# GMC-DRL/MetaBox

Hardware: AMD Instinct MI355X
Metric: env-steps/sec (instances x gens/s), RLEPSO bbob-easy d=10 (higher is better)
Workload: dtype f64

## Files before the change

include/mbx.h:

```cpp
#ifndef MBX_H
#define MBX_H

#include <stddef.h>
#include <stdint.h>

#ifdef __cplusplus
extern "C" {
#endif

#define MBX_OK            0
#define MBX_E_ARG        -1
#define MBX_E_HIP        -2
#define MBX_E_UNSUPPORTED -3
#define MBX_E_NOMEM      -4

#define MBX_KIND_PROTEIN 100

#define MBX_NOISE_NONE    0
#define MBX_NOISE_GAUSS   1
#define MBX_NOISE_UNIFORM 2
#define MBX_NOISE_CAUCHY  3

typedef struct mbx_problem_desc {
    int32_t func_id;
// ... 134 lines not shown
    const float* d_weights;
    int32_t n_floats;
    float min_sigma, max_sigma;
} mbx_gleet_actor;
int mbx_gleet_policy(mbx_batch* b, const mbx_gleet_actor* net, const double* d_state, float* d_actions, float* d_mu_sigma, void* stream);

int mbx_qlpso_rollout(mbx_batch* b, const double* d_q_table, int n_steps, int32_t* d_actions_out, double* d_state_out,
                      double* d_reward_out, uint8_t* d_done_out, void* stream);

int mbx_debug_math(int op, const double* d_x, const double* d_y, double* d_out, int n, void* stream);

int mbx_debug_rlepso_draws(uint64_t seed, int gen, int episode, int np, int dim, double* d_out, void* stream);

int mbx_batch_launch_info(const mbx_batch* b, int32_t out[4]);

int mbx_debug_clock_probe(uint64_t* d_out, int n_samples, int sleep_units, void* stream);
int mbx_debug_clock_mark(uint64_t* d_out2, void* stream);
int mbx_debug_clock_slots(mbx_batch* b, uint64_t* d_slots2);

const char* mbx_last_error(void);
const char* mbx_version(void);

#ifdef __cplusplus
}
#endif
#endif
```

metabox_amd/_abi.py:

```python
import ctypes as C
import os

import numpy as np

_HERE = os.path.dirname(os.path.abspath(__file__))
LIB_PATH = os.environ.get('MBX_LIB') or os.path.join(_HERE, 'csrc', 'libmbx.so')

c_double_p = C.POINTER(C.c_double)


class ProblemDesc(C.Structure):
    _fields_ = [('func_id', C.c_int32), ('kind', C.c_int32), ('dim', C.c_int32), ('n_peaks', C.c_int32),
                ('noise_kind', C.c_int32), ('reserved', C.c_int32),
                ('bias', C.c_double), ('lb', C.c_double), ('ub', C.c_double), ('pen_coef', C.c_double),
                ('s', C.c_double * 4), ('noise_a', C.c_double), ('noise_b', C.c_double),
                ('dshift', c_double_p), ('m1', c_double_p), ('m2', c_double_p),
                ('v0', c_double_p), ('v1', c_double_p), ('v2', c_double_p),
                ('py', c_double_p), ('pc', c_double_p), ('pw', c_double_p)]


class AlgoCfg(C.Structure):
    _fields_ = [('algo', C.c_int32), ('np', C.c_int32), ('dim', C.c_int32), ('max_fes', C.c_int32),
                ('log_interval', C.c_int32), ('n_logpoint', C.c_int32), ('early_stop', C.c_int32),
                ('n_group', C.c_int32), ('flags', C.c_uint32)]
# ... 52 lines not shown
    keep = []
    for i, d in enumerate(descs):
        st, k = pack_desc(d)
        arr[i] = st
        keep.extend(k)
    return arr, keep


_lib = None


class MbxError(RuntimeError):
    pass


def load_lib():
    global _lib
    if _lib is not None:
        return _lib
    if not os.path.exists(LIB_PATH) and not os.environ.get('MBX_LIB'):
        import shutil
        import subprocess
        if shutil.which('hipcc') or os.path.exists('/opt/rocm/bin/hipcc'):
            subprocess.call(['make', '-C', os.path.join(_HERE, 'csrc'), '-s'])
    if not os.path.exists(LIB_PATH):
        raise MbxError(f'{LIB_PATH} is missing: build it with `python -c "import __graft_entry__ as g; g.build()"` '
                       f'(hipcc --offload-arch=gfx950). metabox_amd has no CPU fallback.')
    lib = C.CDLL(LIB_PATH)
    vp, i32, u64, i64 = C.c_void_p, C.c_int32, C.c_uint64, C.c_int64
    proto = {
# ... 18 lines not shown
        'mbx_lde_policy': (C.c_int, [vp, C.POINTER(LstmPolicy), vp, vp, vp, vp, vp, vp]),
        'mbx_ddqn_qnet': (C.c_int, [vp, C.POINTER(QNet), vp, vp, vp, vp]),
        'mbx_rlepso_policy_table_rows': (C.c_int, [vp]),
        'mbx_rlepso_policy_table': (C.c_int, [vp, C.POINTER(GaussMlp), vp, vp]),
        'mbx_rlepso_act_step': (C.c_int, [vp, vp, vp, vp, vp, vp, vp]),
        'mbx_rlepso_rollout_resident': (C.c_int, [vp]),
        'mbx_rlepso_rollout': (C.c_int, [vp, vp, C.c_int, vp, vp, vp, vp, vp, vp, vp, vp]),
        'mbx_lde_rollout_resident': (C.c_int, [vp]),
        'mbx_lde_rollout': (C.c_int, [vp, C.POINTER(LstmPolicy), vp, vp, vp, C.c_int, vp, vp, vp, vp, vp, vp, vp, vp]),
        'mbx_rlpso_rollout': (C.c_int, [vp, C.POINTER(GaussMlp), C.c_int, vp, vp, vp, vp, vp]),
        'mbx_qlpso_rollout': (C.c_int, [vp, vp, C.c_int, vp, vp, vp, vp, vp]),
        'mbx_gleet_policy': (C.c_int, [vp, C.POINTER(GleetActor), vp, vp, vp, vp]),
        'mbx_debug_math': (C.c_int, [C.c_int, vp, vp, vp, C.c_int, vp]),
        'mbx_debug_rlepso_draws': (C.c_int, [C.c_uint64, C.c_int, C.c_int, C.c_int, C.c_int, vp, vp]),
        'mbx_batch_launch_info': (C.c_int, [vp, C.POINTER(C.c_int32)]),
        'mbx_instance_state_doubles': (i64, [vp]),
        'mbx_debug_read_state': (C.c_int, [vp, C.c_int, c_double_p]),
        'mbx_debug_write_state': (C.c_int, [vp, C.c_int, c_double_p]),
        'mbx_debug_clock_probe': (C.c_int, [vp, C.c_int, C.c_int, vp]),
        'mbx_debug_clock_mark': (C.c_int, [vp, vp]),
        'mbx_debug_clock_slots': (C.c_int, [vp, vp]),
        'mbx_batch_rebind': (C.c_int, [vp, vp, vp]),
        'mbx_read_public': (C.c_int, [vp, C.c_int, c_double_p, vp]),
        'mbx_last_error': (C.c_char_p, []),
        'mbx_version': (C.c_char_p, []),
    }
    for name, (res, args) in proto.items():
        fn = getattr(lib, name)
        fn.restype = res
        fn.argtypes = args
    _lib = lib
    return lib


EXPORTED_SYMBOLS = ('mbx_suite_create', 'mbx_suite_destroy', 'mbx_suite_size', 'mbx_suite_optimum', 'mbx_suite_close_pairs', 'mbx_eval', 'mbx_state_dim', 'mbx_action_dim',
                    'mbx_tape_stride', 'mbx_batch_create', 'mbx_batch_destroy', 'mbx_batch_flags', 'mbx_set_tape', 'mbx_reset', 'mbx_step', 'mbx_results',
                    'mbx_gauss_policy', 'mbx_lde_policy', 'mbx_ddqn_qnet', 'mbx_rlepso_policy_table_rows', 'mbx_rlepso_policy_table', 'mbx_rlepso_act_step',
                    'mbx_rlepso_rollout_resident', 'mbx_rlepso_rollout', 'mbx_lde_rollout_resident', 'mbx_lde_rollout', 'mbx_rlpso_rollout',
                    'mbx_qlpso_rollout', 'mbx_gleet_policy', 'mbx_debug_math', 'mbx_debug_rlepso_draws', 'mbx_batch_launch_info', 'mbx_instance_state_doubles',
                    'mbx_debug_read_state', 'mbx_debug_write_state', 'mbx_debug_clock_probe', 'mbx_debug_clock_mark', 'mbx_debug_clock_slots',
                    'mbx_batch_rebind', 'mbx_read_public', 'mbx_last_error', 'mbx_version')


def check(rc):
    if rc != 0:
        msg = load_lib().mbx_last_error()
        raise MbxError(f'mbx error {rc}: {msg.decode() if msg else "?"}')
```

metabox_amd/csrc/mbx.hip:

```cpp
#include <hip/hip_runtime.h>

#include <cmath>
#include <cstdarg>
#include <cstdio>
#include <cstring>
#include <algorithm>
#include <memory>
#include <string>
#include <vector>

#include "mbx_device.hpp"
#include "mbx_rlepso.hpp"
#include "mbx_lde.hpp"
#ifndef MBX_LDE100_STEP_THREADS
#define MBX_LDE100_STEP_THREADS 512
#endif
#ifndef MBX_LDE50_STEP_THREADS
#define MBX_LDE50_STEP_THREADS 256
#endif
#include "mbx_ddqn.hpp"
#include "mbx_rs.hpp"
#include "mbx_policy.hpp"
#include "mbx_lstm_policy.hpp"
#include "mbx_lde_run.hpp"
// ... 935 lines not shown
}

extern "C" int mbx_rlepso_rollout_resident(const mbx_batch* b)
{
    if (!b) return fail(MBX_E_ARG, "mbx_rlepso_rollout_resident: null batch");
    if (b->cfg.algo != MBX_ALGO_RLEPSO) return 0;
    return (b->fixed_geometry == 1 || b->fixed_geometry == 2 || b->fixed_geometry == 7 || b->fixed_geometry == 8 || b->fixed_geometry == 10) && !b->rollout_per_generation ? 1 : 0;
}

__global__ void k_sum_rewards(double* __restrict__ acc, const double* __restrict__ r, int n, int first)
{
    const int i = blockIdx.x * blockDim.x + threadIdx.x;
    if (i < n) acc[i] = first ? r[i] : acc[i] + r[i];
}

static int launch_rlepso_run(mbx_batch* b, const float* d_table, int rows, int n_gens, const RunOut& out, hipStream_t stream)
{
#define MBX_RUN_LAUNCH(T, ...) hipLaunchKernelGGL((k_rlepso_run<T, __VA_ARGS__>), dim3(b->B), dim3(T), b->lds_bytes, stream, make_params(b), d_table, rows, n_gens, out)
    if (b->fixed_geometry == 1) { if (b->fdr_fast) MBX_RUN_LAUNCH(MBX_RUN10_THREADS, 100, 10, 5, false); else MBX_RUN_LAUNCH(MBX_RUN10_THREADS, 100, 10, 5, true); }
    else if (b->fixed_geometry == 2) { if (b->fdr_fast) MBX_RUN_LAUNCH(1024, 128, 40, 5, false); else MBX_RUN_LAUNCH(1024, 128, 40, 5, true); }
    else if (b->fixed_geometry == 7) MBX_RUN_LAUNCH(512, 100, 30, 5, true);
    else if (b->fixed_geometry == 8) MBX_RUN_LAUNCH(256, 100, 12, 5, true);
    else if (b->fixed_geometry == 10) MBX_RUN_LAUNCH(1024, 100, 40, 5, true);
    else return fail(MBX_E_UNSUPPORTED, "k_rlepso_run: no instantiation for this geometry");
#undef MBX_RUN_LAUNCH
    HIP_TRY(hipGetLastError());
    return MBX_OK;
}

extern "C" int mbx_rlepso_rollout(mbx_batch* b, const float* d_table, int n_gens, float* d_traj_actions, double* d_traj_state,
                                  double* d_traj_reward, uint8_t* d_traj_done, double* d_state_out, double* d_reward_out,
                                  uint8_t* d_done_out, void* stream)
{
// ... 230 lines not shown
    b->d_clk = (unsigned long long*)d_slots2;
    return MBX_OK;
}

extern "C" int mbx_batch_launch_info(const mbx_batch* b, int32_t out[4])
{
    if (!b || !out) return fail(MBX_E_ARG, "mbx_batch_launch_info: bad arguments");
    out[0] = b->threads; out[1] = (int32_t)b->lds_bytes; out[2] = b->fixed_geometry; out[3] = (int32_t)b->state_stride;
    if (b->cfg.algo == MBX_ALGO_LDE && b->fixed_geometry == 3) out[0] = MBX_LDE50_STEP_THREADS;
    if (b->cfg.algo == MBX_ALGO_DEDDQN) {
        out[0] = kDqStepThreads; out[1] = (int32_t)(dq_lds_doubles(1, b->cfg.np, b->cfg.dim) * sizeof(double));
    }
    return MBX_OK;
}

extern "C" int mbx_debug_math(int op, const double* d_x, const double* d_y, double* d_out, int n, void* stream)
{
    if (op < 0 || op > 6 || !d_x || !d_out || n < 0 || ((op == 4 || op == 6) && !d_y)) return fail(MBX_E_ARG, "mbx_debug_math: bad arguments");
    if (n) hipLaunchKernelGGL(k_debug_math, dim3((n + 255) / 256), dim3(256), 0, (hipStream_t)stream, op, d_x, d_y, d_out, n);
    HIP_TRY(hipGetLastError());
    return MBX_OK;
}

extern "C" int64_t mbx_instance_state_doubles(const mbx_batch* b)
{
    if (!b) return fail(MBX_E_ARG, "null batch");
    return geom_of(b->cfg).state_doubles;
}

extern "C" int mbx_debug_read_state(mbx_batch* b, int instance, double* host_out)
// ... 44 lines not shown
```

metabox_amd/csrc/mbx_device.hpp:

```cpp
#pragma once
#include <type_traits>
#include <hip/hip_runtime.h>
#include <stdint.h>

#include "../../include/mbx.h"
#include "../../include/mbx_layout.h"
#include "mbx_math.hpp"

namespace mbx {

#ifdef MBX_NOINLINE_MATH
#define MBX_MATH __device__ __noinline__
#else
#define MBX_MATH __device__ __forceinline__
#endif
#ifdef MBX_LIBM_MATH
MBX_MATH double m_pow(double a, double b) { return pow(a, b); }
MBX_MATH double m_sin(double a) { return sin(a); }
MBX_MATH double m_cos(double a) { return cos(a); }
MBX_MATH double m_exp(double a) { return exp(a); }
MBX_MATH double m_log(double a) { return log(a); }
#else
MBX_MATH double m_pow(double a, double b) { return fm::pow_fast(a, b); }
MBX_MATH double m_sin(double a) { return fm::sincos_fast<false>(a); }
// ... 195 lines not shown
__device__ __forceinline__ double asy1(double x, double beta_lin)
{
    return x > 0. ? m_pow(x, 1. + beta_lin * sqrt(x)) : x;
}

__device__ __forceinline__ double pen_row(const double* x, int D, double ub)
{
    double s = 0.;
    for (int d = 0; d < D; ++d) {
        const double t = fmax(0., fabs(x[d]) - ub);
        s += t * t;
    }
    return s;
}

__host__ __device__ inline long long eval_t_doubles(int n, int D)
{
    long long t = (long long)n * D;
    if (t < 17ll * D) t = 17ll * D;
    if (t < 8ll * n) t = 8ll * n;
    return (t + 1) & ~1ll;
}

struct EvalLds {
    const double* X;
    double *Z, *T;
    double *M1T, *M2T;
    double *DSH, *V0, *V1, *V2;
    double* F;
    int z_doubles = 0;
};
// ... 837 lines not shown
```

metabox_amd/csrc/mbx_rlepso.hpp:

```cpp
#pragma once
#include "mbx_device.hpp"

namespace mbx {

struct BatchParams {
    const DevProblem* problems;
    const int32_t* problem_idx;
    const uint64_t* seeds;
    double* state;
    int64_t state_stride;
    const double* tape;
    int64_t tape_stride;
    const int32_t* order;
    const double* pci;
    int32_t NP, D, max_fes, log_interval, n_logpoint, early_stop, n_group, B;
    int64_t sc_off;
    unsigned long long* clk;
};

template <class PT>
__device__ __forceinline__ bool log_and_terminate(const BatchParams& bp, const PT& P, double fes, double gbest, int& log_index,
                                                  int& cost_len, double* __restrict__ cost)
{
    if (fes >= (double)log_index * bp.log_interval) { log_index += 1; cost[cost_len++] = gbest; }
    bool done = fes >= bp.max_fes;
    if (!isnan(P.optimum) && bp.early_stop) done = done || gbest <= 1e-8;
    if (done) {
        if (cost_len >= bp.n_logpoint + 1) cost[cost_len - 1] = gbest;
        else cost[cost_len++] = gbest;
    }
    return done;
}

struct RlLds {
    double *PB, *X, *Z, *T, *M1T, *M2T, *DSH, *V0, *V1, *V2, *PBC, *NC, *PNI, *CMUT, *R1, *R2, *GB, *COEF, *RED;
    int *IMPR, *MASK, *RANK;
    uint8_t* KB;
    uint16_t* FL;
    int* FLN;
    double* NCS;
    int zd;
    __device__ __forceinline__ EvalLds eval() const { return EvalLds{X, Z, T, M1T, M2T, DSH, V0, V1, V2, NC, zd}; }
};

__host__ __device__ inline int64_t align2(int64_t n) { return (n + 1) & ~(int64_t)1; }

__host__ __device__ inline int64_t rl_aux_doubles(int NP, int D) { const int64_t NE = (int64_t)NP * D; return ((NE + 15) / 16 * 16 + 16 + 2 * NE + 7) / 8; }

__host__ __device__ inline int64_t rl_z_doubles(int NP, int D)
{
    const int64_t NE = align2((int64_t)NP * D);
    int64_t need = 3 * align2(NP) + 96 + rl_aux_doubles(NP, D);
    if (need < 2 * kThreads) need = 2 * kThreads;
    if (D == 12 && need < 4 * 4 * 100) need = 4 * 4 * 100;
    return align2(NE > need ? NE : need);
}

#ifndef MBX_RUN_KC40
#define MBX_RUN_KC40 8
#endif
#ifndef MBX_RUN_KC30
#define MBX_RUN_KC30 0
#endif
__host__ __device__ constexpr int rl_run_matvec_chunk(int D) { return D == 40 ? MBX_RUN_KC40 : D == 30 ? MBX_RUN_KC30 : 0; }

__host__ __device__ constexpr bool rl_maps_in_lds(int NP, int D) { return !(NP == 100 && D == 30); }

// ... 25 lines not shown
    L.V0 = p; p += align2(D);
    L.V1 = p; p += align2(D);
    L.V2 = p; p += align2(D);
    L.PBC = p; p += P;
    L.NC = p; p += P;
    L.PNI = p; p += P;
    L.CMUT = p; p += P;
    L.GB = p; p += align2(D);
    L.RED = p; p += 16;
    L.IMPR = (int*)p; p += align2((P + 1) / 2);
    L.MASK = (int*)p; p += align2((P + 1) / 2);
    L.RANK = (int*)p;
    return L;
}

__device__ __forceinline__ void rl_commit(const RlLds& L, int NP, int D, bool stagnation, double& gbest, int& gbest_idx,
                                          double* __restrict__ gPB, double* __restrict__ gCC)
{
    const int tid = threadIdx.x;
    for (int i = tid; i < NP; i += MBX_NT) {
        const double nc = L.NC[i];
        if (stagnation) L.PNI[i] = nc < gCC[i] ? 0. : L.PNI[i] + 1;
        const int impr = nc < L.PBC[i];
        if (impr) L.PBC[i] = nc;
        L.IMPR[i] = impr;
        gCC[i] = nc;
    }
    double cbv; int cb;
    block_argmin(L.NC, NP, L.RED, cbv, cb);
    const bool better = cbv < gbest;
// ... 291 lines not shown
        if (others[q]) {
            double qb = aw[q] / bw[q];
            int ib = ORDER[kb[q]];
            for (int k = 0; k < nless; ++k) {
                const double a = NC[k] - fi, b = fabs(PB[k * D + d0 + q] - pp[q]) + 1e-5, pr = aw[q] * b;
                if (__builtin_fma(a, bw[q], -pr) <= pr * -0x1p-49 && k != kw[q] && !(a == aw[q] && b == bw[q])) {
                    const double qk = a / b;
                    const int ik = ORDER[k];
                    if (qk < qb || (qk == qb && ik < ib)) { qb = qk; ib = ik; kb[q] = k; }
                }
            }
        }
    }
}

template <int W, int UN, bool TIE, int THREADS>
__device__ __forceinline__ void fdr_pass(const RlLds& L, const int* ORDER, const int* NLESS, int NP, int D, int tid, double range, unsigned long long* cnt = nullptr)
{
    const int DW = D / W, NI = NP * DW;
    const FastDiv fw(DW);
    uint32_t mine = 0;
    for (int base = 0, pass = 0; base < NI; base += THREADS, ++pass) {
        const int lim = base + THREADS < NI ? base + THREADS : NI;
        const int ps = (pass & 1) ? lim - 1 - tid : base + tid;
        if (ps >= base && ps < lim) {
            const int rk = fw.div(ps), d0 = W * (ps - rk * DW);
            int kb[W];
            const bool tie = fdr_exact<W, UN, TIE>(L, D, rk, d0, NLESS[ORDER[rk]], kb, range);
#pragma unroll
            for (int q = 0; q < W; ++q) L.KB[rk * D + d0 + q] = (uint8_t)kb[q];
#ifdef MBX_FDR_COUNT
            if (cnt) { atomicAdd(cnt + 3, 1ull); if (tie) atomicAdd(cnt + 2, 1ull); }
#endif
            if (TIE && tie) { L.FL[atomicAdd(L.FLN, 1)] = (uint16_t)ps; mine |= 1u << (pass & 31); }
        }
    }
    __syncthreads();
    if constexpr (TIE) {
        const int n = *L.FLN;
        if (n > 0 && (n <= MBX_FDR_OWN_AT || NI > 32 * THREADS)) {
            for (int c = tid >> 6; c < W * n; c += THREADS / 64) {
                const int ps = L.FL[c / W], rk = fw.div(ps), d = W * (ps - rk * DW) + c % W;
                const int kbest = fdr_settle(L, ORDER, D, rk, d, NLESS[ORDER[rk]], L.KB[rk * D + d], cnt);
                if ((tid & 63) == 0) L.KB[rk * D + d] = (uint8_t)kbest;
            }
            __syncthreads();
        } else if (n > 0) {
            for (int base = 0, pass = 0; mine != 0u; base += THREADS, ++pass, mine >>= 1) {
                if (!(mine & 1u)) continue;
                const int lim = base + THREADS < NI ? base + THREADS : NI;
                const int ps = (pass & 1) ? lim - 1 - tid : base + tid, rk = fw.div(ps), d0 = W * (ps - rk * DW);
// ... 337 lines not shown
        if (done_out) done_out[b] = done ? 1 : 0;
    }
    MBX_PHASE(8);
}

struct RunOut {
    float* traj_actions;
    double* traj_state;
    double* traj_reward;
    uint8_t* traj_done;
    double* state_out;
    double* reward_out;
    uint8_t* done_out;
};

#ifndef MBX_RUN_WAVES
#define MBX_RUN_WAVES MBX_RL_WAVES
#endif
template <int THREADS, int NPC, int DC, int GC, int KIND, int NOISE, bool TIE, class ARGS>
__device__ __forceinline__ void rl_run_body(ARGS ar)
{
    const int n_gens = ar().n_gens;
    static_assert(NPC > 0 && DC > 0 && GC > 0 && (DC & 1) == 0 && NPC <= THREADS, "k_rlepso_run: compile-time geometry, even D, NP <= THREADS");
    constexpr int NP = NPC, D = DC, G = GC, HD = D / 2, NI = NP * HD, IT = (NI + THREADS - 1) / THREADS, A = 7 * G;
    extern __shared__ __attribute__((aligned(16))) double smem[];
    const int b = ar().bp.order[blockIdx.x], tid0 = threadIdx.x, tid = tid0;
    double* S = ar().bp.state + (int64_t)b * ar().bp.state_stride;
    double* sc = S + MBX_RLEPSO_ST_SCALARS(NP, D);
    const int64_t B = ar().bp.B;

    if (sc[MBX_SC_DONE] != 0.) {
        const double st = sc[MBX_SC_FES] / ar().bp.max_fes;
        for (int g = tid; g < n_gens; g += THREADS) {
            if (ar().out.traj_state) ar().out.traj_state[g * B + b] = st;
            if (ar().out.traj_reward) ar().out.traj_reward[g * B + b] = 0.;
            if (ar().out.traj_done) ar().out.traj_done[g * B + b] = 1;
        }
        if (tid == 0) {
            if (ar().out.state_out) ar().out.state_out[b] = st;
            if (ar().out.reward_out) ar().out.reward_out[b] = 0.;
            if (ar().out.done_out) ar().out.done_out[b] = 1;
        }
        return;
    }
    unsigned long long clk_c0 = 0, clk_r0 = 0;
    const bool clocked = ar().bp.clk != nullptr && tid0 == 0;
    if (clocked) { clk_c0 = __builtin_amdgcn_s_memtime(); clk_r0 = __builtin_amdgcn_s_memrealtime(); }
    ConstProblem& P = *(ConstProblem*)(ar().bp.problems + ar().bp.problem_idx[b]);
    const RlLds L = rl_carve(smem, NP, D, rl_maps_in_lds(NPC, DC));
    int gen = (int)sc[MBX_SC_GEN];
    const uint64_t seed = ar().bp.seeds[b];
    const uint32_t episode = (uint32_t)(int)sc[MBX_SC_EPISODE];
    const double lb = P.lb, ub = P.ub, vmax = 0.1 * (ub - lb);
    double gbest = sc[MBX_SC_GBEST];
    int gbest_idx = (int)sc[MBX_SC_GBEST_IDX];
    double fes = sc[MBX_SC_FES];
    int log_index = (int)sc[MBX_SC_LOG_INDEX], cost_len = (int)sc[MBX_SC_COST_LEN];
    double* cost = sc + MBX_NSCALAR;
    double ret = 0.;
    int n_reinit = 0;

    double* gPos = S + MBX_RLEPSO_ST_POS(NP, D);
    double* gVel = S + MBX_RLEPSO_ST_VEL(NP, D);
    double* gPB = S + MBX_RLEPSO_ST_PBPOS(NP, D);
    double vel[IT][2], pbp[IT][2], cc = 0.;
#pragma unroll
    for (int j = 0; j < IT; ++j) {
        const int it = tid + j * THREADS;
        vel[j][0] = vel[j][1] = pbp[j][0] = pbp[j][1] = 0.;
        if (it < NI) {
            const double2 v2 = *(const double2*)(gVel + 2 * it), p2 = *(const double2*)(gPB + 2 * it);
            vel[j][0] = v2.x; vel[j][1] = v2.y; pbp[j][0] = p2.x; pbp[j][1] = p2.y;
            *(double2*)(L.X + 2 * it) = *(const double2*)(gPos + 2 * it);
        }
    }
    if (tid < NP) {
        L.PBC[tid] = S[MBX_RLEPSO_ST_PBEST(NP, D) + tid];
        L.PNI[tid] = S[MBX_RLEPSO_ST_PNI(NP, D) + tid];
        cc = S[MBX_RLEPSO_ST_CCOST(NP, D) + tid];
    }
    if (tid < D) L.GB[tid] = S[MBX_RLEPSO_ST_GBPOS(NP, D) + tid];
    stage_problem<eval_dc(DC), eval_md(DC) == 0, ConstProblem>(P, L.eval());
    constexpr int per_group = NP / G;
    const FastDiv fg(per_group), fh(HD);
    int* ORDER = L.IMPR;
    int* NLESS = L.MASK;
    int* RANK = L.RANK;
    float* ACT = (float*)L.R1;
    int* EQC = (int*)(L.RED + 14);

    auto commit = [&](bool stagnation, int tid) {
        if (tid < NP) {
            const double nc = L.NC[tid];
            if (stagnation) L.PNI[tid] = nc < cc ? 0. : L.PNI[tid] + 1;
            const int impr = nc < L.PBC[tid];
            if (impr) L.PBC[tid] = nc;
            L.IMPR[tid] = impr;
            cc = nc;
        }
        double cbv; int cb;
        block_argmin(L.NC, NP, L.RED, cbv, cb);
        const bool better = cbv < gbest;
        if (better) { gbest = cbv; gbest_idx = cb; }
#pragma unroll
        for (int j = 0; j < IT; ++j) {
            const int it = tid + j * THREADS;
            if (it < NI && L.IMPR[fh.div(it)]) { const double2 x2 = *(const double2*)(L.X + 2 * it); pbp[j][0] = x2.x; pbp[j][1] = x2.y; }
        }
        if (better && tid < D) L.GB[tid] = L.X[cb * D + tid];
        __syncthreads();
    };

    bool done = false;
    int g = 0;
    __syncthreads();
    for (; g < n_gens && !done; ++g) {
        int tid = tid0;
        asm volatile("" : "+v"(tid));
        gen += 1;
        const Rng rng{(uint32_t)seed, (uint32_t)(seed >> 32), (uint32_t)gen, episode, true};
        const double pre_gbest = gbest;
        if (tid < A) {
            int row = (int)fes;
            row = row < ar().table_rows ? row : ar().table_rows - 1;
            const float* ms = ar().policy_table + (int64_t)row * 2 * A;
            const float a = sample_action(rng, tid, ms[tid], ms[A + tid], MBX_POLICY_RLEPSO);
            ACT[tid] = a;
            if (ar().out.traj_actions) ar().out.traj_actions[((int64_t)g * B + b) * A + tid] = a;
        }
        if (tid < NP) { NLESS[tid] = 0; ORDER[tid] = tid; }
        if (tid == 0) { *EQC = 0; *L.FLN = 0; }
        __syncthreads();
        if (tid < G) {
            const float* a = ACT + tid * G;
            const float cm = a[0] * 0.01f;
            const float wv = a[1] * 0.8f + 0.1f;
            float den = a[3] + a[4];
            den = den + a[5]; den = den + a[6]; den = den + 1e-5f;
            float scale = 1.f / den;
            scale = scale * a[2]; scale = scale * 8.f;
            double* c = L.COEF + tid * 6;
            c[0] = (double)cm; c[1] = (double)wv;
            c[2] = (double)(scale * a[3]); c[3] = (double)(scale * a[4]);
            c[4] = (double)(scale * a[5]); c[5] = (double)(scale * a[6]);
        }
        {
            constexpr int parts = THREADS / NP > 0 ? THREADS / NP : 1;
            for (int w = tid; w < parts * NP; w += THREADS) {
                const int part = w / NP, i = w - part * NP;
                const int j0 = part * NP / parts, j1 = (part + 1) * NP / parts;
                const double fi = L.PBC[i];
                int nless = 0;
#ifndef MBX_ABLATE_RANK
#pragma unroll 5
                for (int j = j0; j < j1; ++j) nless += L.PBC[j] < fi;
#else
                if (part == 0) nless = i;
#endif
                atomicAdd(&NLESS[i], nless);
            }
        }
        __syncthreads();
        if (tid < NP) {
            const int i = tid, gi = fg.div(i);
            L.CMUT[i] = gi < G ? L.COEF[gi * 6] * L.PNI[i] : 0.;
            const U4 w = rng.draw((uint32_t)i, MBX_SITE_PART);
            L.R1[i] = u53(w.x, w.y); L.R2[i] = u53(w.z, w.w);
            const int rank = NLESS[i];
            RANK[i] = rank;
            ORDER[rank] = i; L.NC[rank] = L.PBC[i]; L.NCS[rank] = L.PBC[i];
        }
        __syncthreads();
        if (tid < NP && ORDER[RANK[tid]] != tid) *EQC = 1;
        auto stage_pbest = [&](int tid) {
#pragma unroll
            for (int j = 0; j < IT; ++j) {
                const int it = tid + j * THREADS;
                if (it < NI) { const int i = fh.div(it), d0 = 2 * (it - i * HD); *(double2*)(L.PB + RANK[i] * D + d0) = double2{pbp[j][0], pbp[j][1]}; }
            }
        };
        stage_pbest(tid);
        __syncthreads();
        if (*EQC) {
            int rank = 0;
            if (tid < NP) {
                const double fi = L.PBC[tid];
                rank = NLESS[tid];
                for (int j = 0; j < tid; ++j) rank += L.PBC[j] == fi;
            }
            __syncthreads();
            if (tid < NP) { RANK[tid] = rank; ORDER[rank] = tid; L.NC[rank] = L.PBC[tid]; L.NCS[rank] = L.PBC[tid]; }
            __syncthreads();
            stage_pbest(tid);
            __syncthreads();
            rl_mark_copies(L, NP, D, tid);
            __syncthreads();
        }
#ifdef MBX_ABLATE_FDR
        for (int e = tid; e < NP * D; e += THREADS) L.KB[e] = 0;
        __syncthreads();
#else
        fdr_pass<2, (DC == 40 ? 2 : MBX_FDR_UNROLL), TIE, THREADS>(L, ORDER, NLESS, NP, D, tid, ub - lb + 1e-5, ar().bp.clk);
#endif
        {
            const MoveCtx mc{L, ar().bp.pci, nullptr, rng, nullptr, nullptr, ORDER, NLESS, RANK, NP, D, G, lb, ub, vmax, fg};
#pragma unroll
            for (int j = 0; j < IT; ++j) {
                const int it = tid + j * THREADS;
                if (it < NI) {
                    const int i = fh.div(it);
                    const double2 c2 = *(const double2*)(L.X + 2 * it);
                    double cur[2] = {c2.x, c2.y};
                    rl_move<2, true>(mc, i, 2 * (it - i * HD), cur, vel[j]);
                }
            }
        }
        __syncthreads();
        population_costs<eval_dc(DC), eval_md(DC), ConstProblem, rl_run_matvec_chunk(DC), KIND, NOISE>(P, L.eval(), NP, rng, nullptr, MBX_SITE_NOISE0_A, MBX_SITE_NOISE0_B);
        fes += NP;
        commit(true, tid);
        int mine = 0;
        if (tid < NP) {
            const U4 w = rng.draw((uint32_t)tid, MBX_SITE_REINIT);
            const double u = u53(w.x, w.y);
            mine = u < L.CMUT[tid] * 0.01 * L.PNI[tid];
            L.MASK[tid] = mine;
        }
        n_reinit = __syncthreads_count(mine);
        if (n_reinit > 0) {
#pragma unroll
            for (int j = 0; j < IT; ++j) {
                const int it = tid + j * THREADS;
                if (it < NI && L.MASK[fh.div(it)]) {
#pragma unroll
                    for (int q = 0; q < 2; ++q) {
                        const int e = 2 * it + q;
                        const U4 w = rng.draw((uint32_t)e, MBX_SITE_ELEM_R);
                        const double up = u53(w.x, w.y), uv = u53(w.z, w.w);
                        L.X[e] = lb + (ub - lb) * up;
                        vel[j][q] = -vmax + (vmax - (-vmax)) * uv;
                    }
                }
            }
            __syncthreads();
            population_costs<eval_dc(DC), eval_md(DC), ConstProblem, rl_run_matvec_chunk(DC), KIND, NOISE>(P, L.eval(), NP, rng, nullptr, MBX_SITE_NOISE1_A, MBX_SITE_NOISE1_B);
            fes += n_reinit;
            commit(false, tid);
        }
        if (fes >= (double)log_index * ar().bp.log_interval) { log_index += 1; if (tid == 0) cost[cost_len] = gbest; cost_len += 1; }
        done = fes >= ar().bp.max_fes;
        if (!isnan(P.optimum) && ar().bp.early_stop) done = done || gbest <= 1e-8;
        if (done) {
            if (cost_len >= ar().bp.n_logpoint + 1) { if (tid == 0) cost[cost_len - 1] = gbest; }
            else { if (tid == 0) cost[cost_len] = gbest; cost_len += 1; }
        }
        const double reward = gbest < pre_gbest ? 1. : -1.;
        ret += reward;
        if (tid == 0) {
            if (ar().out.traj_state) ar().out.traj_state[g * B + b] = fes / ar().bp.max_fes;
            if (ar().out.traj_reward) ar().out.traj_reward[g * B + b] = reward;
            if (ar().out.traj_done) ar().out.traj_done[g * B + b] = done ? 1 : 0;
        }
    }
#pragma unroll
    for (int j = 0; j < IT; ++j) {
        const int it = tid + j * THREADS;
        if (it < NI) {
            *(double2*)(gPos + 2 * it) = *(const double2*)(L.X + 2 * it);
            *(double2*)(gVel + 2 * it) = double2{vel[j][0], vel[j][1]};
            *(double2*)(gPB + 2 * it) = double2{pbp[j][0], pbp[j][1]};
        }
    }
    if (tid < NP) {
        S[MBX_RLEPSO_ST_PBEST(NP, D) + tid] = L.PBC[tid];
        S[MBX_RLEPSO_ST_PNI(NP, D) + tid] = L.PNI[tid];
        S[MBX_RLEPSO_ST_CCOST(NP, D) + tid] = cc;
    }
    if (tid < D) S[MBX_RLEPSO_ST_GBPOS(NP, D) + tid] = L.GB[tid];
    const double st = fes / ar().bp.max_fes;
    for (int t = g + tid; t < n_gens; t += THREADS) {
        if (ar().out.traj_state) ar().out.traj_state[t * B + b] = st;
        if (ar().out.traj_reward) ar().out.traj_reward[t * B + b] = 0.;
        if (ar().out.traj_done) ar().out.traj_done[t * B + b] = 1;
    }
    if (tid == 0) {
        sc[MBX_SC_GBEST] = gbest; sc[MBX_SC_FES] = fes; sc[MBX_SC_LOG_INDEX] = log_index; sc[MBX_SC_COST_LEN] = cost_len;
        sc[MBX_SC_DONE] = done ? 1. : 0.; sc[MBX_SC_RETURN] += ret; sc[MBX_SC_GEN] = gen;
        sc[MBX_SC_GBEST_IDX] = gbest_idx; sc[MBX_SC_REINIT] = n_reinit > 0 ? 1. : 0.;
        if (ar().out.state_out) ar().out.state_out[b] = st;
        if (ar().out.reward_out) ar().out.reward_out[b] = ret;
// ... 74 lines not shown
```

metabox_amd/suite.py:

```python
import ctypes as C

import numpy as np
import torch

from . import _abi


def _require_gpu():
    if not torch.cuda.is_available():
        raise _abi.MbxError('metabox_amd needs a ROCm GPU (MI355X); there is no CPU fallback for the hot path.')


def _ptr(t):
    return C.c_void_p(t.data_ptr()) if t is not None else C.c_void_p()


def _stream():
    return C.c_void_p(torch.cuda.current_stream().cuda_stream)


class Suite:

    def __init__(self, problems):
        _require_gpu()
# ... 273 lines not shown
        _abi.check(self.lib.mbx_debug_read_state(self._h, int(instance), out.ctypes.data_as(_abi.c_double_p)))
        return out

    def write_state(self, instance, block):
        n = int(self.lib.mbx_instance_state_doubles(self._h))
        block = np.ascontiguousarray(block, dtype=np.float64)
        assert block.shape == (n,)
        _abi.check(self.lib.mbx_debug_write_state(self._h, int(instance), block.ctypes.data_as(_abi.c_double_p)))

    def launch_info(self):
        import ctypes as C
        out = (C.c_int32 * 4)()
        _abi.check(self.lib.mbx_batch_launch_info(self._h, out))
        return {'threads': out[0], 'lds_bytes': out[1], 'fixed_geometry': out[2], 'state_doubles': out[3]}

    def close(self):
        if getattr(self, '_h', None):
            self.lib.mbx_batch_destroy(self._h)
            self._h = None

    def __del__(self):
        try:
            self.close()
        except Exception:
            pass
```

Baseline: 35.67 million.

## Compact LDS and park velocity/pbest in global memory for six RLEPSO workgroups per CU

For the 256-thread, NP=100, D=10 resident RLEPSO kernel, this adds a compact LDS carve-out. It drops the matrix maps, CMUT and the double PNI array, and stores integer tables in the free tail of Z. Velocity and personal-best positions move out of registers into global memory, and the velocity fetch is hooked into the FDR pass so it overlaps. The waves-per-EU hint rises to 6, aiming for six workgroups per CU to raise occupancy. In exchange it adds global memory traffic each generation and re-reads maps from global memory instead of LDS, and it adds an occupancy-query diagnostic API.

```diff
diff --git a/include/mbx.h b/include/mbx.h
--- a/include/mbx.h
+++ b/include/mbx.h
@@ -172,6 +172,8 @@
 
 int mbx_batch_launch_info(const mbx_batch* b, int32_t out[4]);
 
+int mbx_rlepso_run_launch_info(const mbx_batch* b, int32_t out[3]);
+
 int mbx_debug_clock_probe(uint64_t* d_out, int n_samples, int sleep_units, void* stream);
 int mbx_debug_clock_mark(uint64_t* d_out2, void* stream);
 int mbx_debug_clock_slots(mbx_batch* b, uint64_t* d_slots2);
diff --git a/metabox_amd/_abi.py b/metabox_amd/_abi.py
--- a/metabox_amd/_abi.py
+++ b/metabox_amd/_abi.py
@@ -90,6 +90,9 @@
     pass
 
 
+_DIAGNOSTICS_SINCE = ('mbx_rlepso_run_launch_info',)
+
+
 def load_lib():
     global _lib
     if _lib is not None:
@@ -138,6 +141,7 @@
         'mbx_debug_math': (C.c_int, [C.c_int, vp, vp, vp, C.c_int, vp]),
         'mbx_debug_rlepso_draws': (C.c_int, [C.c_uint64, C.c_int, C.c_int, C.c_int, C.c_int, vp, vp]),
         'mbx_batch_launch_info': (C.c_int, [vp, C.POINTER(C.c_int32)]),
+        'mbx_rlepso_run_launch_info': (C.c_int, [vp, C.POINTER(C.c_int32)]),
         'mbx_instance_state_doubles': (i64, [vp]),
         'mbx_debug_read_state': (C.c_int, [vp, C.c_int, c_double_p]),
         'mbx_debug_write_state': (C.c_int, [vp, C.c_int, c_double_p]),
@@ -150,6 +154,8 @@
         'mbx_version': (C.c_char_p, []),
     }
     for name, (res, args) in proto.items():
+        if name in _DIAGNOSTICS_SINCE and os.environ.get('MBX_LIB') and not hasattr(lib, name):
+            continue
         fn = getattr(lib, name)
         fn.restype = res
         fn.argtypes = args
@@ -161,7 +167,8 @@
                     'mbx_tape_stride', 'mbx_batch_create', 'mbx_batch_destroy', 'mbx_batch_flags', 'mbx_set_tape', 'mbx_reset', 'mbx_step', 'mbx_results',
                     'mbx_gauss_policy', 'mbx_lde_policy', 'mbx_ddqn_qnet', 'mbx_rlepso_policy_table_rows', 'mbx_rlepso_policy_table', 'mbx_rlepso_act_step',
                     'mbx_rlepso_rollout_resident', 'mbx_rlepso_rollout', 'mbx_lde_rollout_resident', 'mbx_lde_rollout', 'mbx_rlpso_rollout',
-                    'mbx_qlpso_rollout', 'mbx_gleet_policy', 'mbx_debug_math', 'mbx_debug_rlepso_draws', 'mbx_batch_launch_info', 'mbx_instance_state_doubles',
+                    'mbx_qlpso_rollout', 'mbx_gleet_policy', 'mbx_debug_math', 'mbx_debug_rlepso_draws', 'mbx_batch_launch_info', 'mbx_rlepso_run_launch_info',
+                    'mbx_instance_state_doubles',
                     'mbx_debug_read_state', 'mbx_debug_write_state', 'mbx_debug_clock_probe', 'mbx_debug_clock_mark', 'mbx_debug_clock_slots',
                     'mbx_batch_rebind', 'mbx_read_public', 'mbx_last_error', 'mbx_version')
 
diff --git a/metabox_amd/csrc/mbx.hip b/metabox_amd/csrc/mbx.hip
--- a/metabox_amd/csrc/mbx.hip
+++ b/metabox_amd/csrc/mbx.hip
@@ -973,9 +973,17 @@
     if (i < n) acc[i] = first ? r[i] : acc[i] + r[i];
 }
 
+static size_t rlepso_run_lds_bytes(const mbx_batch* b)
+{
+    if (b->fixed_geometry == 1 && rl_run_compact(MBX_RUN10_THREADS, 100, 10))
+        return (size_t)rl_run_lds_doubles(100, 10) * sizeof(double) + (b->lds_bytes - (size_t)rl_lds_doubles(100, 10, true) * sizeof(double));
+    return b->lds_bytes;
+}
+
 static int launch_rlepso_run(mbx_batch* b, const float* d_table, int rows, int n_gens, const RunOut& out, hipStream_t stream)
 {
-#define MBX_RUN_LAUNCH(T, ...) hipLaunchKernelGGL((k_rlepso_run<T, __VA_ARGS__>), dim3(b->B), dim3(T), b->lds_bytes, stream, make_params(b), d_table, rows, n_gens, out)
+    const size_t run_lds = rlepso_run_lds_bytes(b);
+#define MBX_RUN_LAUNCH(T, ...) hipLaunchKernelGGL((k_rlepso_run<T, __VA_ARGS__>), dim3(b->B), dim3(T), run_lds, stream, make_params(b), d_table, rows, n_gens, out)
     if (b->fixed_geometry == 1) { if (b->fdr_fast) MBX_RUN_LAUNCH(MBX_RUN10_THREADS, 100, 10, 5, false); else MBX_RUN_LAUNCH(MBX_RUN10_THREADS, 100, 10, 5, true); }
     else if (b->fixed_geometry == 2) { if (b->fdr_fast) MBX_RUN_LAUNCH(1024, 128, 40, 5, false); else MBX_RUN_LAUNCH(1024, 128, 40, 5, true); }
     else if (b->fixed_geometry == 7) MBX_RUN_LAUNCH(512, 100, 30, 5, true);
@@ -1236,6 +1244,27 @@
     return MBX_OK;
 }
 
+extern "C" int mbx_rlepso_run_launch_info(const mbx_batch* b, int32_t out[3])
+{
+    if (!b || !out) return fail(MBX_E_ARG, "mbx_rlepso_run_launch_info: bad arguments");
+    if (mbx_rlepso_rollout_resident(b) != 1) return fail(MBX_E_UNSUPPORTED, "mbx_rlepso_run_launch_info: the batch's rollout does not take the resident kernel");
+    const void* k = nullptr;
+    int threads = 0;
+#define MBX_RUN_KERNEL(T, ...) do { k = (const void*)k_rlepso_run<T, __VA_ARGS__>; threads = T; } while (0)
+    if (b->fixed_geometry == 1) { if (b->fdr_fast) MBX_RUN_KERNEL(MBX_RUN10_THREADS, 100, 10, 5, false); else MBX_RUN_KERNEL(MBX_RUN10_THREADS, 100, 10, 5, true); }
+    else if (b->fixed_geometry == 2) { if (b->fdr_fast) MBX_RUN_KERNEL(1024, 128, 40, 5, false); else MBX_RUN_KERNEL(1024, 128, 40, 5, true); }
+    else if (b->fixed_geometry == 7) MBX_RUN_KERNEL(512, 100, 30, 5, true);
+    else if (b->fixed_geometry == 8) MBX_RUN_KERNEL(256, 100, 12, 5, true);
+    else if (b->fixed_geometry == 10) MBX_RUN_KERNEL(1024, 100, 40, 5, true);
+    else return fail(MBX_E_UNSUPPORTED, "k_rlepso_run: no instantiation for this geometry");
+#undef MBX_RUN_KERNEL
+    const size_t lds = rlepso_run_lds_bytes(b);
+    int per_cu = 0;
+    HIP_TRY(hipOccupancyMaxActiveBlocksPerMultiprocessor(&per_cu, k, threads, lds));
+    out[0] = threads; out[1] = (int32_t)lds; out[2] = per_cu;
+    return MBX_OK;
+}
+
 extern "C" int mbx_debug_math(int op, const double* d_x, const double* d_y, double* d_out, int n, void* stream)
 {
     if (op < 0 || op > 6 || !d_x || !d_out || n < 0 || ((op == 4 || op == 6) && !d_y)) return fail(MBX_E_ARG, "mbx_debug_math: bad arguments");
diff --git a/metabox_amd/csrc/mbx_device.hpp b/metabox_amd/csrc/mbx_device.hpp
--- a/metabox_amd/csrc/mbx_device.hpp
+++ b/metabox_amd/csrc/mbx_device.hpp
@@ -233,7 +233,7 @@
     return s;
 }
 
-__host__ __device__ inline long long eval_t_doubles(int n, int D)
+__host__ __device__ constexpr long long eval_t_doubles(int n, int D)
 {
     long long t = (long long)n * D;
     if (t < 17ll * D) t = 17ll * D;
diff --git a/metabox_amd/csrc/mbx_rlepso.hpp b/metabox_amd/csrc/mbx_rlepso.hpp
--- a/metabox_amd/csrc/mbx_rlepso.hpp
+++ b/metabox_amd/csrc/mbx_rlepso.hpp
@@ -35,6 +35,7 @@
 struct RlLds {
     double *PB, *X, *Z, *T, *M1T, *M2T, *DSH, *V0, *V1, *V2, *PBC, *NC, *PNI, *CMUT, *R1, *R2, *GB, *COEF, *RED;
     int *IMPR, *MASK, *RANK;
+    int* PNII = nullptr;
     uint8_t* KB;
     uint16_t* FL;
     int* FLN;
@@ -43,14 +44,16 @@
     __device__ __forceinline__ EvalLds eval() const { return EvalLds{X, Z, T, M1T, M2T, DSH, V0, V1, V2, NC, zd}; }
 };
 
-__host__ __device__ inline int64_t align2(int64_t n) { return (n + 1) & ~(int64_t)1; }
-
-__host__ __device__ inline int64_t rl_aux_doubles(int NP, int D) { const int64_t NE = (int64_t)NP * D; return ((NE + 15) / 16 * 16 + 16 + 2 * NE + 7) / 8; }
-
-__host__ __device__ inline int64_t rl_z_doubles(int NP, int D)
+__host__ __device__ constexpr int64_t align2(int64_t n) { return (n + 1) & ~(int64_t)1; }
+
+__host__ __device__ constexpr int64_t rl_aux_doubles(int NP, int D) { const int64_t NE = (int64_t)NP * D; return ((NE + 15) / 16 * 16 + 16 + 2 * NE + 7) / 8; }
+
+__host__ __device__ constexpr int64_t rl_z_move_doubles(int NP, int D) { return 3 * align2(NP) + 96 + rl_aux_doubles(NP, D); }
+
+__host__ __device__ constexpr int64_t rl_z_doubles(int NP, int D)
 {
     const int64_t NE = align2((int64_t)NP * D);
-    int64_t need = 3 * align2(NP) + 96 + rl_aux_doubles(NP, D);
+    int64_t need = rl_z_move_doubles(NP, D);
     if (need < 2 * kThreads) need = 2 * kThreads;
     if (D == 12 && need < 4 * 4 * 100) need = 4 * 4 * 100;
     return align2(NE > need ? NE : need);
@@ -106,6 +109,49 @@
     return L;
 }
 
+#ifndef MBX_RUN_COMPACT
+#define MBX_RUN_COMPACT 1
+#endif
+#ifndef MBX_LDS_GRANULE
+#define MBX_LDS_GRANULE 1280
+#endif
+__host__ __device__ constexpr bool rl_run_compact(int THREADS, int NP, int D) { return MBX_RUN_COMPACT && THREADS == 256 && NP == 100 && D == 10; }
+
+__host__ __device__ constexpr int64_t rl_run_lds_doubles(int NP, int D)
+{
+    const int64_t NE = align2((int64_t)NP * D), P = align2(NP);
+    return eval_t_doubles(NP, D) + NE + rl_z_doubles(NP, D) + 5 * align2(D) + 2 * P + 16 + align2((P + 1) / 2);
+}
+
+__device__ __forceinline__ RlLds rl_carve_run(double* base, int NP, int D)
+{
+    const int64_t NE = align2((int64_t)NP * D), SC = rl_z_doubles(NP, D), P = align2(NP), TS = eval_t_doubles(NP, D), IT = align2((P + 1) / 2);
+    RlLds L;
+    double* p = base;
+    L.PB = p; L.T = p; p += TS;
+    L.X = p; p += NE;
+    L.Z = p; L.zd = (int)SC;
+    L.R1 = p; L.R2 = p + P; L.COEF = p + 2 * P;
+    L.NCS = p + 2 * P + 96;
+    L.KB = (uint8_t*)(p + 3 * P + 96);
+    L.FLN = (int*)(L.KB + ((int64_t)NP * D + 15) / 16 * 16);
+    L.FL = (uint16_t*)(L.FLN + 4);
+    double* tail = p + rl_z_move_doubles(NP, D);
+    L.MASK = (int*)tail; L.RANK = (int*)(tail + IT); L.IMPR = (int*)(tail + 2 * IT);
+    p += SC;
+    L.M1T = nullptr; L.M2T = nullptr; L.PNI = nullptr; L.CMUT = nullptr;
+    L.DSH = p; p += align2(D);
+    L.V0 = p; p += align2(D);
+    L.V1 = p; p += align2(D);
+    L.V2 = p; p += align2(D);
+    L.GB = p; p += align2(D);
+    L.PBC = p; p += P;
+    L.NC = p; p += P;
+    L.RED = p; p += 16;
+    L.PNII = (int*)p;
+    return L;
+}
+
 __device__ __forceinline__ void rl_commit(const RlLds& L, int NP, int D, bool stagnation, double& gbest, int& gbest_idx,
                                           double* __restrict__ gPB, double* __restrict__ gCC)
 {
@@ -427,8 +473,10 @@
     }
 }
 
-template <int W, int UN, bool TIE, int THREADS>
-__device__ __forceinline__ void fdr_pass(const RlLds& L, const int* ORDER, const int* NLESS, int NP, int D, int tid, double range, unsigned long long* cnt = nullptr)
+struct FdrNoHook { __device__ __forceinline__ void operator()() const {} };
+template <int W, int UN, bool TIE, int THREADS, class HOOK = FdrNoHook>
+__device__ __forceinline__ void fdr_pass(const RlLds& L, const int* ORDER, const int* NLESS, int NP, int D, int tid, double range, unsigned long long* cnt = nullptr,
+                                         HOOK after_scan = HOOK())
 {
     const int DW = D / W, NI = NP * DW;
     const FastDiv fw(DW);
@@ -448,6 +496,7 @@
             if (TIE && tie) { L.FL[atomicAdd(L.FLN, 1)] = (uint16_t)ps; mine |= 1u << (pass & 31); }
         }
     }
+    after_scan();
     __syncthreads();
     if constexpr (TIE) {
         const int n = *L.FLN;
@@ -815,15 +864,27 @@
     uint8_t* done_out;
 };
 
+#ifndef MBX_RUN_SIX
+#define MBX_RUN_SIX 1
+#endif
 #ifndef MBX_RUN_WAVES
-#define MBX_RUN_WAVES MBX_RL_WAVES
-#endif
+#define MBX_RUN_WAVES __attribute__((amdgpu_waves_per_eu(MBX_RUN_SIX && rl_run_compact(THREADS, NPC, DC) ? 6 : THREADS == 256 ? 5 : 4)))
+#endif
+#ifndef MBX_RUN_PARK
+#define MBX_RUN_PARK 1
+#endif
+__host__ __device__ constexpr bool rl_run_parked(int THREADS, int NP, int D) { return MBX_RUN_PARK && THREADS == 256 && NP == 100 && D == 10; }
 template <int THREADS, int NPC, int DC, int GC, int KIND, int NOISE, bool TIE, class ARGS>
 __device__ __forceinline__ void rl_run_body(ARGS ar)
 {
     const int n_gens = ar().n_gens;
     static_assert(NPC > 0 && DC > 0 && GC > 0 && (DC & 1) == 0 && NPC <= THREADS, "k_rlepso_run: compile-time geometry, even D, NP <= THREADS");
     constexpr int NP = NPC, D = DC, G = GC, HD = D / 2, NI = NP * HD, IT = (NI + THREADS - 1) / THREADS, A = 7 * G;
+    constexpr bool PARK = rl_run_parked(THREADS, NPC, DC);
+    constexpr bool COMPACT = rl_run_compact(THREADS, NPC, DC);
+    constexpr int MDR = COMPACT ? DC : eval_md(DC);
+    static_assert(!COMPACT || rl_z_move_doubles(NPC, DC) + 3 * align2((align2(NPC) + 1) / 2) <= rl_z_doubles(NPC, DC), "the integer tables must fit the free tail of Z");
+    static_assert(!COMPACT || rl_run_lds_doubles(NPC, DC) * 8 <= 163840 / 6 / MBX_LDS_GRANULE * MBX_LDS_GRANULE, "six workgroups per CU");
     extern __shared__ __attribute__((aligned(16))) double smem[];
     const int b = ar().bp.order[blockIdx.x], tid0 = threadIdx.x, tid = tid0;
     double* S = ar().bp.state + (int64_t)b * ar().bp.state_stride;
@@ -848,7 +909,9 @@
     const bool clocked = ar().bp.clk != nullptr && tid0 == 0;
     if (clocked) { clk_c0 = __builtin_amdgcn_s_memtime(); clk_r0 = __builtin_amdgcn_s_memrealtime(); }
     ConstProblem& P = *(ConstProblem*)(ar().bp.problems + ar().bp.problem_idx[b]);
-    const RlLds L = rl_carve(smem, NP, D, rl_maps_in_lds(NPC, DC));
+    const RlLds L = COMPACT ? rl_carve_run(smem, NP, D) : rl_carve(smem, NP, D, rl_maps_in_lds(NPC, DC));
+    auto pni = [&](int i) -> double { if constexpr (COMPACT) return (double)L.PNII[i]; else return L.PNI[i]; };
+    auto set_pni = [&](int i, double v) { if constexpr (COMPACT) L.PNII[i] = (int)v; else L.PNI[i] = v; };
     int gen = (int)sc[MBX_SC_GEN];
     const uint64_t seed = ar().bp.seeds[b];
     const uint32_t episode = (uint32_t)(int)sc[MBX_SC_EPISODE];
@@ -870,18 +933,20 @@
         const int it = tid + j * THREADS;
         vel[j][0] = vel[j][1] = pbp[j][0] = pbp[j][1] = 0.;
         if (it < NI) {
-            const double2 v2 = *(const double2*)(gVel + 2 * it), p2 = *(const double2*)(gPB + 2 * it);
-            vel[j][0] = v2.x; vel[j][1] = v2.y; pbp[j][0] = p2.x; pbp[j][1] = p2.y;
+            if constexpr (!PARK) {
+                const double2 v2 = *(const double2*)(gVel + 2 * it), p2 = *(const double2*)(gPB + 2 * it);
+                vel[j][0] = v2.x; vel[j][1] = v2.y; pbp[j][0] = p2.x; pbp[j][1] = p2.y;
+            }
             *(double2*)(L.X + 2 * it) = *(const double2*)(gPos + 2 * it);
         }
     }
     if (tid < NP) {
         L.PBC[tid] = S[MBX_RLEPSO_ST_PBEST(NP, D) + tid];
-        L.PNI[tid] = S[MBX_RLEPSO_ST_PNI(NP, D) + tid];
+        set_pni(tid, S[MBX_RLEPSO_ST_PNI(NP, D) + tid]);
         cc = S[MBX_RLEPSO_ST_CCOST(NP, D) + tid];
     }
     if (tid < D) L.GB[tid] = S[MBX_RLEPSO_ST_GBPOS(NP, D) + tid];
-    stage_problem<eval_dc(DC), eval_md(DC) == 0, ConstProblem>(P, L.eval());
+    stage_problem<eval_dc(DC), MDR == 0, ConstProblem>(P, L.eval());
     constexpr int per_group = NP / G;
     const FastDiv fg(per_group), fh(HD);
     int* ORDER = L.IMPR;
@@ -893,7 +958,7 @@
     auto commit = [&](bool stagnation, int tid) {
         if (tid < NP) {
             const double nc = L.NC[tid];
-            if (stagnation) L.PNI[tid] = nc < cc ? 0. : L.PNI[tid] + 1;
+            if (stagnation) set_pni(tid, nc < cc ? 0. : pni(tid) + 1);
             const int impr = nc < L.PBC[tid];
             if (impr) L.PBC[tid] = nc;
             L.IMPR[tid] = impr;
@@ -906,7 +971,11 @@
 #pragma unroll
         for (int j = 0; j < IT; ++j) {
             const int it = tid + j * THREADS;
-            if (it < NI && L.IMPR[fh.div(it)]) { const double2 x2 = *(const double2*)(L.X + 2 * it); pbp[j][0] = x2.x; pbp[j][1] = x2.y; }
+            if (it < NI && L.IMPR[fh.div(it)]) {
+                const double2 x2 = *(const double2*)(L.X + 2 * it);
+                if constexpr (PARK) *(double2*)(gPB + 2 * it) = x2;
+                else { pbp[j][0] = x2.x; pbp[j][1] = x2.y; }
+            }
         }
         if (better && tid < D) L.GB[tid] = L.X[cb * D + tid];
         __syncthreads();
@@ -932,6 +1001,14 @@
         if (tid < NP) { NLESS[tid] = 0; ORDER[tid] = tid; }
         if (tid == 0) { *EQC = 0; *L.FLN = 0; }
         __syncthreads();
+        double2 pq[IT];
+        if constexpr (PARK) {
+#pragma unroll
+            for (int j = 0; j < IT; ++j) {
+                const int it = tid + j * THREADS;
+                pq[j] = it < NI ? *(const double2*)(gPB + 2 * it) : double2{0., 0.};
+            }
+        }
         if (tid < G) {
             const float* a = ACT + tid * G;
             const float cm = a[0] * 0.01f;
@@ -962,9 +1039,11 @@
             }
         }
         __syncthreads();
+        double cmut = 0.;
         if (tid < NP) {
             const int i = tid, gi = fg.div(i);
-            L.CMUT[i] = gi < G ? L.COEF[gi * 6] * L.PNI[i] : 0.;
+            cmut = gi < G ? L.COEF[gi * 6] * pni(i) : 0.;
+            if constexpr (!COMPACT) L.CMUT[i] = cmut;
             const U4 w = rng.draw((uint32_t)i, MBX_SITE_PART);
             L.R1[i] = u53(w.x, w.y); L.R2[i] = u53(w.z, w.w);
             const int rank = NLESS[i];
@@ -977,7 +1056,10 @@
 #pragma unroll
             for (int j = 0; j < IT; ++j) {
                 const int it = tid + j * THREADS;
-                if (it < NI) { const int i = fh.div(it), d0 = 2 * (it - i * HD); *(double2*)(L.PB + RANK[i] * D + d0) = double2{pbp[j][0], pbp[j][1]}; }
+                if (it < NI) {
+                    const int i = fh.div(it), d0 = 2 * (it - i * HD);
+                    *(double2*)(L.PB + RANK[i] * D + d0) = PARK ? pq[j] : double2{pbp[j][0], pbp[j][1]};
+                }
             }
         };
         stage_pbest(tid);
@@ -992,16 +1074,34 @@
             __syncthreads();
             if (tid < NP) { RANK[tid] = rank; ORDER[rank] = tid; L.NC[rank] = L.PBC[tid]; L.NCS[rank] = L.PBC[tid]; }
             __syncthreads();
+            if constexpr (PARK) {
+#pragma unroll
+                for (int j = 0; j < IT; ++j) {
+                    const int it = tid + j * THREADS;
+                    if (it < NI) pq[j] = *(const double2*)(gPB + 2 * it);
+                }
+            }
             stage_pbest(tid);
             __syncthreads();
             rl_mark_copies(L, NP, D, tid);
             __syncthreads();
         }
+        double2 vq[IT];
+        auto fetch_vel = [&]() {
+            if constexpr (PARK) {
+#pragma unroll
+                for (int j = 0; j < IT; ++j) {
+                    const int it = tid + j * THREADS;
+                    vq[j] = it < NI ? *(const double2*)(gVel + 2 * it) : double2{0., 0.};
+                }
+            }
+        };
 #ifdef MBX_ABLATE_FDR
         for (int e = tid; e < NP * D; e += THREADS) L.KB[e] = 0;
+        fetch_vel();
         __syncthreads();
 #else
-        fdr_pass<2, (DC == 40 ? 2 : MBX_FDR_UNROLL), TIE, THREADS>(L, ORDER, NLESS, NP, D, tid, ub - lb + 1e-5, ar().bp.clk);
+        fdr_pass<2, (DC == 40 ? 2 : MBX_FDR_UNROLL), TIE, THREADS>(L, ORDER, NLESS, NP, D, tid, ub - lb + 1e-5, ar().bp.clk, fetch_vel);
 #endif
         {
             const MoveCtx mc{L, ar().bp.pci, nullptr, rng, nullptr, nullptr, ORDER, NLESS, RANK, NP, D, G, lb, ub, vmax, fg};
@@ -1012,19 +1112,24 @@
                     const int i = fh.div(it);
                     const double2 c2 = *(const double2*)(L.X + 2 * it);
                     double cur[2] = {c2.x, c2.y};
-                    rl_move<2, true>(mc, i, 2 * (it - i * HD), cur, vel[j]);
+                    if constexpr (PARK) {
+                        double vl[2] = {vq[j].x, vq[j].y};
+                        rl_move<2, true>(mc, i, 2 * (it - i * HD), cur, vl);
+                        *(double2*)(gVel + 2 * it) = double2{vl[0], vl[1]};
+                    } else rl_move<2, true>(mc, i, 2 * (it - i * HD), cur, vel[j]);
                 }
             }
         }
         __syncthreads();
-        population_costs<eval_dc(DC), eval_md(DC), ConstProblem, rl_run_matvec_chunk(DC), KIND, NOISE>(P, L.eval(), NP, rng, nullptr, MBX_SITE_NOISE0_A, MBX_SITE_NOISE0_B);
+        population_costs<eval_dc(DC), MDR, ConstProblem, rl_run_matvec_chunk(DC), KIND, NOISE>(P, L.eval(), NP, rng, nullptr, MBX_SITE_NOISE0_A, MBX_SITE_NOISE0_B);
         fes += NP;
         commit(true, tid);
         int mine = 0;
         if (tid < NP) {
             const U4 w = rng.draw((uint32_t)tid, MBX_SITE_REINIT);
             const double u = u53(w.x, w.y);
-            mine = u < L.CMUT[tid] * 0.01 * L.PNI[tid];
+            if constexpr (!COMPACT) cmut = L.CMUT[tid];
+            mine = u < cmut * 0.01 * pni(tid);
             L.MASK[tid] = mine;
         }
         n_reinit = __syncthreads_count(mine);
@@ -1033,18 +1138,21 @@
             for (int j = 0; j < IT; ++j) {
                 const int it = tid + j * THREADS;
                 if (it < NI && L.MASK[fh.div(it)]) {
+                    double nv[2];
 #pragma unroll
                     for (int q = 0; q < 2; ++q) {
                         const int e = 2 * it + q;
                         const U4 w = rng.draw((uint32_t)e, MBX_SITE_ELEM_R);
                         const double up = u53(w.x, w.y), uv = u53(w.z, w.w);
                         L.X[e] = lb + (ub - lb) * up;
-                        vel[j][q] = -vmax + (vmax - (-vmax)) * uv;
+                        nv[q] = -vmax + (vmax - (-vmax)) * uv;
                     }
+                    if constexpr (PARK) *(double2*)(gVel + 2 * it) = double2{nv[0], nv[1]};
+                    else { vel[j][0] = nv[0]; vel[j][1] = nv[1]; }
                 }
             }
             __syncthreads();
-            population_costs<eval_dc(DC), eval_md(DC), ConstProblem, rl_run_matvec_chunk(DC), KIND, NOISE>(P, L.eval(), NP, rng, nullptr, MBX_SITE_NOISE1_A, MBX_SITE_NOISE1_B);
+            population_costs<eval_dc(DC), MDR, ConstProblem, rl_run_matvec_chunk(DC), KIND, NOISE>(P, L.eval(), NP, rng, nullptr, MBX_SITE_NOISE1_A, MBX_SITE_NOISE1_B);
             fes += n_reinit;
             commit(false, tid);
         }
@@ -1068,13 +1176,15 @@
         const int it = tid + j * THREADS;
         if (it < NI) {
             *(double2*)(gPos + 2 * it) = *(const double2*)(L.X + 2 * it);
-            *(double2*)(gVel + 2 * it) = double2{vel[j][0], vel[j][1]};
-            *(double2*)(gPB + 2 * it) = double2{pbp[j][0], pbp[j][1]};
+            if constexpr (!PARK) {
+                *(double2*)(gVel + 2 * it) = double2{vel[j][0], vel[j][1]};
+                *(double2*)(gPB + 2 * it) = double2{pbp[j][0], pbp[j][1]};
+            }
         }
     }
     if (tid < NP) {
         S[MBX_RLEPSO_ST_PBEST(NP, D) + tid] = L.PBC[tid];
-        S[MBX_RLEPSO_ST_PNI(NP, D) + tid] = L.PNI[tid];
+        S[MBX_RLEPSO_ST_PNI(NP, D) + tid] = pni(tid);
         S[MBX_RLEPSO_ST_CCOST(NP, D) + tid] = cc;
     }
     if (tid < D) S[MBX_RLEPSO_ST_GBPOS(NP, D) + tid] = L.GB[tid];
diff --git a/metabox_amd/suite.py b/metabox_amd/suite.py
--- a/metabox_amd/suite.py
+++ b/metabox_amd/suite.py
@@ -311,6 +311,12 @@
         _abi.check(self.lib.mbx_batch_launch_info(self._h, out))
         return {'threads': out[0], 'lds_bytes': out[1], 'fixed_geometry': out[2], 'state_doubles': out[3]}
 
+    def run_launch_info(self):
+        import ctypes as C
+        out = (C.c_int32 * 3)()
+        _abi.check(self.lib.mbx_rlepso_run_launch_info(self._h, out))
+        return {'threads': out[0], 'lds_bytes': out[1], 'workgroups_per_cu': out[2]}
+
     def close(self):
         if getattr(self, '_h', None):
             self.lib.mbx_batch_destroy(self._h)
```

Result: slower. 33.50 million (-6.1%).
